# joshua16266261/self-play-ai

Hardware: AMD Instinct MI355X
Metric: MCTS sims/sec + self-play games/sec, Connect4 800 sims/move, 1/2/4/8 GPU (higher is better)
Workload: dtype bf16

## Files before the change

### self-play-ai_amd/csrc/net_c4.hip

```cpp
#include <algorithm>
#include <cmath>
#include <cstdlib>
#include <cstring>

#include "spai_internal.h"

namespace spai {
namespace {

typedef __bf16 bf16x8 __attribute__((ext_vector_type(8)));
typedef float f32x4 __attribute__((ext_vector_type(4)));
typedef float f32x2 __attribute__((ext_vector_type(2)));
typedef __bf16 bf16x2 __attribute__((ext_vector_type(2)));
typedef short i16x2 __attribute__((ext_vector_type(2)));

constexpr int kHid = 64;
constexpr int kS = 8;
constexpr int kP = kS * c4::kCells;
__host__ __device__ constexpr int npt_of(int S) { return (S * c4::kCells + 15) / 16; }
constexpr int kWaves = 4;
#ifdef SPAI_W8
constexpr int kPhysWaves = 8;
#else
constexpr int kPhysWaves = 4;
#endif
constexpr int kThreads = kPhysWaves * 64;
constexpr int kStemThreads = kWaves * 64;
constexpr int kKStepsRes = 18;
constexpr int kHeadC = 35;
constexpr int kPolIn = 32 * c4::kCells;
constexpr int kValIn = 3 * c4::kCells;

constexpr int kZ = 0;
constexpr int kX = 256;
constexpr int kZ1 = kX + kP * 128;
constexpr int kY = kZ1 + 256;
constexpr int kHC = 36;
constexpr int kLinFeat = kHC * 42;
constexpr int kLinK = 1536;
constexpr int kLinKSteps = kLinK / 32;
constexpr int kLinPitch = kLinK + 16;
constexpr int kLinHalves = 2;
constexpr int kLinBSteps = kLinKSteps / kLinHalves;
constexpr int kH = kY;
constexpr int kHBytes = kP * 128;
constexpr int kB = kH + kHBytes;
constexpr int kL = kB + kS * 16;
constexpr int kMaxBlocks = 20;
constexpr int kBiasFloats = kHid + 2 * kMaxBlocks * kHid + kHid;
constexpr int kBias = kL + kWaves * kLinHalves * 64 * 4;
constexpr int kBiasPer = (kBiasFloats + kStemThreads - 1) / kStemThreads;
constexpr int kPlanes = kBias + kBiasFloats * 4;
constexpr int kPlaneRow = 34;
constexpr int kWStem = kPlanes + kS * kPlaneRow * 8;
constexpr int kTab = kWStem + 4 * 64 * 16;
constexpr int kLinWPer = kLinBSteps / kWaves;
#ifdef SPAI_W8
constexpr int kSRun = 5;
constexpr int kSplitMaxN = 14;
constexpr int kPart = kTab + 42 * 16;
constexpr int kLdsBytes = kPart + kWaves * kSplitMaxN * 1024;
#else
constexpr int kSRun = kS;
constexpr int kLdsBytes = kTab + 42 * 16;
#endif
#ifdef SPAI_DIAG_KSTEP
constexpr int kStamps = 48;
#else
constexpr int kStamps = 24;
#endif
static_assert(kS * kLinPitch * 2 <= kHBytes, "head features fit in Y");
static_assert(kLdsBytes <= 160 * 1024, "LDS budget");

struct NetParams {
    const uint4 *w_stem;
    const uint4 *w_res;
    const uint4 *w_head;
    const float *b_conv;
    const uint4 *w_lin;
    const float *b_pol;
    const float *b_val;
    const uint4 *geo;
    const uint4 *lane_geo;
    unsigned long long *stamps;
    int blocks;
};

#ifdef SPAI_DIAG_HEAD
constexpr bool kDiagHead = true;
#else
constexpr bool kDiagHead = false;
#endif
#ifdef SPAI_DIAG_ENTRY
constexpr bool kDiagEntry = true;
#else
[[maybe_unused]] constexpr bool kDiagEntry = false;
#endif
__device__ __forceinline__ void stamp(const NetParams &P, int wave, int lane, int k) {
#ifdef SPAI_DIAG
    if (P.stamps && lane == 0 && wave >= 0) P.stamps[((size_t)blockIdx.x * kWaves + wave) * kStamps + k] = __builtin_amdgcn_s_memtime();
#endif
}
__device__ __forceinline__ void stamp_real(const NetParams &P, int wave, int lane, int k) {
#ifdef SPAI_DIAG
    if (P.stamps && lane == 0 && wave >= 0)
        P.stamps[((size_t)blockIdx.x * kWaves + wave) * kStamps + k] = __builtin_amdgcn_s_memrealtime();
#endif
}

__device__ __forceinline__ bf16x8 as_bf16x8(uint4 v) { return __builtin_bit_cast(bf16x8, v); }

__device__ __forceinline__ uint32_t pack_bf16x2(float a, float b) {
    return __builtin_bit_cast(uint32_t, __builtin_convertvector((f32x2){a, b}, bf16x2));
}

__device__ __forceinline__ uint32_t pack_relu_bf16x2(float a, float b) {
    const i16x2 h = __builtin_bit_cast(i16x2, __builtin_convertvector((f32x2){a, b}, bf16x2));
    return __builtin_bit_cast(uint32_t, __builtin_elementwise_max(h, (i16x2){0, 0}));
}

constexpr uint8_t kCellOrder[9][42] = {
    {0, 0, 0, 0, 0, 0, 0, 0, 0, 0, 0, 0, 0, 0, 0, 0, 0, 0, 0, 0, 0, 0, 0, 0, 0, 0, 0, 0, 0, 0, 0, 0, 0, 0, 0, 0, 0, 0, 0, 0, 0, 0},
    {0, 1, 2, 3, 4, 5, 6, 7, 8, 9, 10, 11, 12, 13, 14, 15, 16, 17, 18, 19, 20, 21, 22, 23, 24, 25, 26, 27, 28, 29, 30, 31, 32, 33, 34, 35, 36, 37, 38, 39, 40, 41},
    {0, 1, 2, 3, 4, 5, 6, 7, 8, 9, 10, 11, 12, 13, 14, 15, 16, 17, 18, 19, 20, 21, 22, 23, 24, 25, 26, 27, 28, 29, 30, 31, 32, 33, 34, 35, 36, 37, 38, 39, 40, 41},
    {0, 1, 2, 3, 4, 5, 6, 7, 8, 9, 10, 11, 12, 13, 14, 15, 16, 17, 18, 19, 20, 21, 22, 23, 24, 25, 26, 27, 28, 29, 30, 31, 32, 33, 34, 35, 36, 37, 38, 39, 40, 41},
    {22, 33, 10, 23, 24, 11, 26, 17, 8, 25, 18, 5, 6, 3, 4, 1, 34, 13, 20, 27, 30, 9, 16, 7, 38, 37, 40, 41, 0, 21, 14, 35, 32, 31, 12, 29, 28, 19, 2, 15, 36, 39},
    {13, 5, 30, 10, 23, 12, 38, 40, 37, 36, 0, 32, 27, 41, 20, 34, 2, 4, 3, 1, 16, 18, 26, 33, 39, 31, 22, 11, 28, 21, 14, 7, 8, 9, 15, 19, 24, 17, 35, 25, 29, 6},
    {37, 20, 40, 33, 22, 13, 25, 24, 35, 39, 38, 7, 10, 32, 19, 17, 27, 34, 41, 8, 16, 11, 36, 12, 2, 0, 4, 6, 26, 28, 1, 29, 30, 3, 15, 9, 31, 5, 23, 18, 21, 14},
    {8, 22, 4, 3, 1, 13, 20, 9, 33, 7, 21, 14, 25, 18, 19, 24, 35, 28, 0, 2, 5, 31, 32, 12, 16, 38, 36, 40, 39, 37, 26, 17, 27, 6, 34, 11, 30, 15, 23, 29, 10, 41},
    {28, 21, 41, 37, 18, 26, 1, 2, 16, 29, 22, 31, 15, 17, 5, 6, 24, 8, 13, 20, 4, 3, 33, 30, 27, 34, 0, 35, 12, 25, 23, 10, 36, 39, 19, 11, 32, 9, 38, 40, 7, 14},
};
__host__ __device__ constexpr uint16_t tap_skip(int S, int t) {
    constexpr uint16_t m1[21] = {0, 0, 0, 0, 0, 0, 0, 0, 0, 0, 0, 0, 0, 0, 0, 0, 0, 0, 0, 0, 0};
    constexpr uint16_t m2[21] = {0, 0, 0, 0, 0, 0, 0, 0, 0, 0, 0, 0, 0, 0, 0, 0, 0, 0, 0, 0, 0};
    constexpr uint16_t m3[21] = {0, 0, 0, 0, 0, 0, 0, 0, 0, 0, 0, 0, 0, 0, 0, 0, 0, 0, 0, 0, 0};
    constexpr uint16_t m4[21] = {0, 0, 0, 7, 292, 0, 448, 73, 0, 0, 448, 0, 0, 0, 0, 0, 0, 0, 0, 0, 0};
    constexpr uint16_t m5[21] = {0, 0, 448, 0, 292, 7, 0, 0, 0, 73, 0, 0, 0, 295, 0, 0, 0, 0, 0, 0, 0};
    constexpr uint16_t m6[21] = {256, 0, 0, 448, 0, 0, 292, 0, 0, 7, 0, 0, 0, 0, 0, 73, 0, 0, 0, 0, 0};
    constexpr uint16_t m7[21] = {0, 7, 4, 0, 73, 0, 0, 73, 7, 0, 0, 448, 448, 0, 292, 0, 0, 0, 484, 0, 0};
    constexpr uint16_t m8[21] = {73, 448, 0, 7, 0, 0, 0, 7, 0, 292, 7, 0, 292, 73, 0, 0, 448, 0, 0, 448, 73};
    return S == 1 ? m1[t] : S == 2 ? m2[t] : S == 3 ? m3[t] : S == 4 ? m4[t] : S == 5 ? m5[t] : S == 6 ? m6[t] : S == 7 ? m7[t] : m8[t];
}
__host__ __device__ constexpr bool cell_major(int S) { return S >= 4; }
__host__ __device__ constexpr int lin_pitch(int S) { return S == 4 ? 1552 : 1544; }
__host__ __device__ constexpr int first_kstep(int S, int t) {
    int tap = 0;
    while ((tap_skip(S, t) >> tap) & 1) ++tap;
    return 2 * tap;
}

#ifndef SPAI_CO_MAJOR_MAX_NPT
#define SPAI_CO_MAJOR_MAX_NPT 8
#endif
#ifndef SPAI_PAIR_MAX_NPT
#define SPAI_PAIR_MAX_NPT 11
#endif
#ifndef SPAI_HEAD_CO_MAJOR_MAX_NPT
#define SPAI_HEAD_CO_MAJOR_MAX_NPT 8
#endif
#ifdef SPAI_DEFER_EPI
constexpr bool kDefer = true;
#else
constexpr bool kDefer = false;
#endif
__host__ __device__ constexpr int kstep_of(int j) { return kDefer ? (j < 9 ? 2 * j : 2 * (j - 9) + 1) : j; }

template <int W, int CT, int NPT>
struct Plan {
    static constexpr int MODE = NPT <= (CT == 3 ? SPAI_HEAD_CO_MAJOR_MAX_NPT : SPAI_CO_MAJOR_MAX_NPT) ? 1
                                : CT == 4 && NPT <= SPAI_PAIR_MAX_NPT                              ? 2
                                                                                                    : 0;
    static constexpr int TT = NPT * CT;
    static constexpr int first = TT * W / 4;
    static constexpr int nr = TT * (W + 1) / 4 - first;
    static constexpr int last = first + nr - 1;
    static constexpr int m = NPT / 2, r = NPT % 2, pj = W >> 1, ph = W & 1;

    static constexpr int n = MODE == 2 ? 2 * m + r : nr;
    static constexpr int C0 = MODE == 2 ? 2 * pj : MODE == 1 ? first / NPT : 0;
    static constexpr int CTL = MODE == 2 ? 2 : MODE == 1 ? last / NPT - C0 + 1 : CT;
    static constexpr int T0 = MODE == 2 ? ph * m
                              : MODE == 1 ? (CTL == 1 ? first % NPT : 0)
                                          : first / CT;
    static constexpr int NT = MODE == 2 ? m + r : MODE == 1 ? (CTL == 1 ? nr : NPT) : last / CT - T0 + 1;
    static constexpr int gpt(int t) { return MODE == 2 && t == m ? NPT - 1 : T0 + t; }
    static constexpr int pt(int i) {
        return MODE == 2 ? (i < 2 * m ? i / 2 : m) : (MODE == 1 ? (first + i) % NPT : (first + i) / CT) - T0;
    }
    static constexpr int co(int i) {
        return MODE == 2 ? (i < 2 * m ? 2 * pj + (i & 1) : 2 * pj + ph)
                         : MODE == 1 ? (first + i) / NPT : (first + i) % CT;
    }
    static constexpr bool DEFER = kDefer && CT == 4 && MODE == 0;
    static constexpr int count_deferred() {
        int c = 0;
        for (int i = 0; i < n; ++i) c += co(i) >= 2;
        return c;
    }
    static constexpr int ND = DEFER ? count_deferred() : 0;
    static constexpr int NDA = ND > 0 ? n : 1;
    static constexpr bool deferred(int i) { return DEFER && co(i) >= 2; }
};

template <int NT>
struct Geo {
    uint32_t rel2[NT][5];
    int epi[NT];
    __device__ __forceinline__ uint32_t b(int t, int tap) const {
        return (tap & 1) ? rel2[t][tap >> 1] >> 16 : rel2[t][tap >> 1] & 0xFFFFu;
    }
};

struct RowCell {
    int s, cell, idx;
};
template <int S>
__device__ __forceinline__ RowCell row_cell(const uint8_t *smem, int p) {
    if (p >= S * c4::kCells) return RowCell{0, -1, 0};
    if constexpr (!cell_major(S)) {
        const int s = p / c4::kCells, cell = p - s * c4::kCells;
        return RowCell{s, cell, cell};
    } else {
        const int idx = p / S;
        return RowCell{p - idx * S, (int)((const uint32_t *)(smem + kTab))[idx * 4], idx};
    }
}

template <int W, int CT, int NPT, int S>
__device__ __forceinline__ void make_geo(const uint8_t *smem, int lane, Geo<Plan<W, CT, NPT>::NT> &g) {
    using PL = Plan<W, CT, NPT>;
    const int col = lane & 15, q = lane >> 4;
#pragma unroll
    for (int t = 0; t < PL::NT; ++t) {
        const int p = PL::gpt(t) * 16 + col;
        if constexpr (!cell_major(S)) {
            const int cell = p % c4::kCells;
            const int h = cell / c4::kCols, w = cell - h * c4::kCols;
#pragma unroll
            for (int tap = 0; tap < 9; ++tap) {
                const int dh = tap / 3 - 1, dw = tap % 3 - 1;
                const int r = p + dh * c4::kCols + dw;
                const bool ok = (unsigned)(h + dh) < (unsigned)c4::kRows && (unsigned)(w + dw) < (unsigned)c4::kCols;
                const int full = r * 128 + ((q ^ (r & 7)) << 4);
                const uint32_t v = (uint32_t)((ok ? full : (full & 255) - 256) + 256);
                if (tap & 1) g.rel2[t][tap >> 1] |= v << 16;
                else g.rel2[t][tap >> 1] = v;
            }
        } else {
            const bool real = p < S * c4::kCells;
            const int idx = real ? p / S : 0, s = p - idx * S;
            const uint4 e = *(const uint4 *)(smem + kTab + idx * 16);
            const int own = p * 128 + ((q ^ (p & 7)) << 4);
#pragma unroll
            for (int tap = 0; tap < 9; ++tap) {
                const uint32_t word = tap < 4 ? e.y : tap < 8 ? e.z : e.w;
                const int nb = (int)((word >> (8 * (tap & 3))) & 255u);
                int v;
                if (real && nb != 255) {
                    const int r = nb * S + s;
                    v = r * 128 + ((q ^ (r & 7)) << 4) + 256;
                } else if (S == 4) {
                    const int r = (((idx ^ (tap / 3 + tap % 3)) & 1) << 2) + s;
                    v = (r * 128 + ((q ^ (r & 7)) << 4)) & 255;
                } else {
                    v = own & 255;
                }
                if (tap & 1) g.rel2[t][tap >> 1] |= (uint32_t)v << 16;
                else g.rel2[t][tap >> 1] = (uint32_t)v;
            }
        }
        g.epi[t] = p * 128 + ((((q >> 1)) ^ (p & 7)) << 4) + ((q & 1) << 3);
    }
}

#ifndef SPAI_GEO_NT
#define SPAI_GEO_NT 8
#endif
constexpr int kGeoNT = SPAI_GEO_NT;
__host__ __device__ constexpr size_t lane_geo_at(int S, int W, int t) {
    return (((size_t)(S - 1) * kWaves + W) * kGeoNT + t) * 64 * 2;
}
constexpr size_t kLaneGeoU4 = lane_geo_at(kS + 1, 0, 0);

template <int W, int NPT, int S>
__device__ __forceinline__ void load_geo(const NetParams &P, int lane, Geo<Plan<W, 4, NPT>::NT> &g,
                                         int (&aux)[Plan<W, 4, NPT>::NT]) {
    constexpr int NT = Plan<W, 4, NPT>::NT;
    static_assert(NT <= kGeoNT, "lane geometry table depth");
    const uint4 *src = P.lane_geo + lane_geo_at(S, W, 0) + 2 * lane;
#pragma unroll
    for (int t = 0; t < NT; ++t) {
        const uint4 a = src[t * 128], b = src[t * 128 + 1];
        g.rel2[t][0] = a.x;
        g.rel2[t][1] = a.y;
        g.rel2[t][2] = a.z;
        g.rel2[t][3] = a.w;
        g.rel2[t][4] = b.x;
        g.epi[t] = (int)b.y;
        aux[t] = (int)b.z;
    }
}

template <int S, int W>
__device__ void geo_init_one(const uint8_t *smem, uint4 *out, int lane) {
    constexpr int NPT = npt_of(S);
    using PL = Plan<W, 4, NPT>;
    Geo<PL::NT> g;
    make_geo<W, 4, NPT, S>(smem, lane, g);
    uint4 *dst = out + lane_geo_at(S, W, 0) + 2 * lane;
    for (int t = 0; t < PL::NT; ++t) {
        const RowCell rc = row_cell<S>(smem, PL::gpt(t) * 16 + (lane & 15));
        const int h = rc.cell / c4::kCols, w = rc.cell - h * c4::kCols;
        const int aux = rc.cell < 0 ? S : rc.s | (w * 7 + h) << 8;
        dst[t * 128] = make_uint4(g.rel2[t][0], g.rel2[t][1], g.rel2[t][2], g.rel2[t][3]);
        dst[t * 128 + 1] = make_uint4(g.rel2[t][4], (uint32_t)g.epi[t], (uint32_t)aux, 0u);
    }
}

template <int S>
__device__ void geo_init_s(const uint8_t *smem, uint4 *out, int W, int lane) {
    if (W == 0) geo_init_one<S, 0>(smem, out, lane);
    else if (W == 1) geo_init_one<S, 1>(smem, out, lane);
    else if (W == 2) geo_init_one<S, 2>(smem, out, lane);
    else geo_init_one<S, 3>(smem, out, lane);
}

__global__ __launch_bounds__(64) void k_geo_init(const uint4 *__restrict__ geo, uint4 *__restrict__ out) {
    __shared__ __attribute__((aligned(16))) uint8_t smem[kLdsBytes];
    const int S = blockIdx.x / kWaves + 1, W = blockIdx.x % kWaves, lane = threadIdx.x;
    if (lane < c4::kCells) ((uint4 *)(smem + kTab))[lane] = geo[S * c4::kCells + lane];
    __syncthreads();
    switch (S) {
    case 1: geo_init_s<1>(smem, out, W, lane); break;
    case 2: geo_init_s<2>(smem, out, W, lane); break;
    case 3: geo_init_s<3>(smem, out, W, lane); break;
    case 4: geo_init_s<4>(smem, out, W, lane); break;
    case 5: geo_init_s<5>(smem, out, W, lane); break;
    case 6: geo_init_s<6>(smem, out, W, lane); break;
    case 7: geo_init_s<7>(smem, out, W, lane); break;
    default: geo_init_s<8>(smem, out, W, lane); break;
    }
}

#ifndef SPAI_FINAL_HINTS
#define SPAI_FINAL_HINTS 1
#endif
#ifndef SPAI_FINAL_FENCE
#define SPAI_FINAL_FENCE 1
#endif
#ifndef SPAI_ISSUE_HINTS
#define SPAI_ISSUE_HINTS 0
#endif
#ifndef SPAI_KSTEP_FENCE
#define SPAI_KSTEP_FENCE 1
#endif
#ifndef SPAI_DA4
#define SPAI_DA4 6
#endif
#ifndef SPAI_DB4
#define SPAI_DB4 2
#endif
#ifndef SPAI_DA8
#ifdef SPAI_FINAL2
#define SPAI_DA8 6
#else
#define SPAI_DA8 3
#endif
#endif
#ifndef SPAI_DB8
#define SPAI_DB8 3
#endif
__host__ __device__ constexpr int a_depth(int S) { return S <= 2 ? 9 : S <= 3 ? 6 : S <= 4 ? SPAI_DA4 : SPAI_DA8; }
__host__ __device__ constexpr int b_depth(int S) { return S <= 2 ? 4 : S <= 3 ? 3 : S <= 4 ? SPAI_DB4 : SPAI_DB8; }

__device__ __forceinline__ uint4 exp_a(const uint4 &src, int lane, int k) {
#ifdef SPAI_EXP_NOA
    (void)src;
    return make_uint4(0x3F803F80u ^ (uint32_t)(lane + k), 0x3F803F80u, 0x3F803F80u, (uint32_t)k);
#else
    (void)lane, (void)k;
    return src;
#endif
}
__device__ __forceinline__ uint4 exp_b(const uint8_t *p, int lane, int k) {
#ifdef SPAI_EXP_NOB
    (void)p;
    return make_uint4(0x3F803F80u ^ (uint32_t)(lane * 3 + k), 0x3F803F80u, 0x3F803F80u, (uint32_t)k);
#else
    (void)lane, (void)k;
    return *(const uint4 *)p;
#endif
}
__device__ __forceinline__ void layer_barrier() {
#ifndef SPAI_EXP_NOBAR
    __syncthreads();
#endif
}

template <int W, int CT, int NPT, int S, int DA, int DB, int EPI, int OUT>
__device__ __forceinline__ void final_tap_epilogue(uint8_t *smem, const Geo<Plan<W, CT, NPT>::NT> &g, int lane,
                                                   const uint4 (&A)[DA][Plan<W, CT, NPT>::CTL],
                                                   const uint4 (&B)[DB][Plan<W, CT, NPT>::NT],
                                                   const f32x4 (&bv)[Plan<W, CT, NPT>::CTL],
                                                   f32x4 (&acc)[Plan<W, CT, NPT>::n],
                                                   const int (&hoff)[Plan<W, CT, NPT>::NT],
                                                   f32x4 (&dacc)[Plan<W, CT, NPT>::NDA]) {
    using PL = Plan<W, CT, NPT>;
    auto defer = [](int i) { return EPI < 3 && PL::deferred(i); };
#ifdef SPAI_EXP_EPI_LAG
    constexpr int n = PL::n, k0 = kKStepsRes - 2, D = SPAI_EXP_EPI_LAG;
#else
    constexpr int n = PL::n, k0 = kKStepsRes - 2, D = 2;
#endif
    static_assert(CT == 4, "fused epilogue: 64-channel layers");
    auto live = [](int t, int ks) { return !((tap_skip(S, PL::gpt(t)) >> (ks >> 1)) & 1); };
    auto task_on = [](int i) { return !(EPI == 3 && PL::co(i) == 3); };
    uint4 id[2];
    uint4 rb[3];
    if (EPI == 2) {
        const int m = lane & 15, q = lane >> 4;
#pragma unroll
        for (int h = 0; h < 2; ++h) {
            const int j = 16 * h + m - 8 * q;
            uint32_t w[4];
#pragma unroll
            for (int e = 0; e < 4; ++e) w[e] = j == 2 * e ? 0x3F80u : j == 2 * e + 1 ? 0x3F800000u : 0u;
            id[h] = make_uint4(w[0], w[1], w[2], w[3]);
        }
#pragma unroll
        for (int i = 0; i < 2 && i < n; ++i)
            rb[i] = *(const uint4 *)(smem + (OUT - 256) + (g.b(PL::pt(i), 4) ^ ((PL::co(i) >> 1) << 6)));
    }
#pragma unroll
    for (int i = 0; i < n + D; ++i) {
        int nm = 0, nv = 0, nw = 0, nrd = 0;
        if (i < n) {
            if (EPI == 2 && i + 2 < n) {
                rb[(i + 2) % 3] = *(const uint4 *)(smem + (OUT - 256) + (g.b(PL::pt(i + 2), 4) ^ ((PL::co(i + 2) >> 1) << 6)));
                ++nrd;
            }
            const int t = PL::gpt(PL::pt(i)), c = PL::co(i) - PL::C0;
#pragma unroll
            for (int j = k0; j < kKStepsRes; ++j) {
                const int ks = kstep_of(j);
                if (task_on(i) && live(PL::pt(i), ks)) {
                    acc[i] = __builtin_amdgcn_mfma_f32_16x16x32_bf16(as_bf16x8(A[j % DA][c]), as_bf16x8(B[j % DB][PL::pt(i)]),
                                                                    ks == first_kstep(S, t) ? bv[c] : acc[i], 0, 0, 0);
                    ++nm;
                }
            }
            if (EPI == 2) {
                acc[i] = __builtin_amdgcn_mfma_f32_16x16x32_bf16(as_bf16x8(id[PL::co(i) & 1]), as_bf16x8(rb[i % 3]), acc[i],
                                                                0, 0, 0);
                ++nm;
            }
        }
        if (i >= D && EPI < 3 && !defer(i - D)) {
            const int j = i - D;
            const int off = OUT + (g.epi[PL::pt(j)] ^ (PL::co(j) << 5));
#if defined(SPAI_EXP_NOEPI) || defined(SPAI_EXP_NOEPI_ALL)
            asm volatile("" ::"a"(acc[j]));
#ifdef SPAI_EXP_NOEPI
            *(uint2 *)(smem + off) = make_uint2(0u, (uint32_t)off);
            nw = 1;
#endif
            nv = 0;
#elif defined(SPAI_EXP_STORE_B128)
            if ((j & 1) == 0) {
                const uint32_t a0 = pack_relu_bf16x2(acc[j][0], acc[j][1]), a1 = pack_relu_bf16x2(acc[j][2], acc[j][3]);
                const int j2 = j + 1 < PL::n ? j + 1 : j;
                const uint32_t b0 = pack_relu_bf16x2(acc[j2][0], acc[j2][1]), b1 = pack_relu_bf16x2(acc[j2][2], acc[j2][3]);
                *(uint4 *)(smem + (off & ~15)) = make_uint4(a0, a1, b0, b1);
                nw = 1;
            }
            nv = 5;
#elif defined(SPAI_EXP_STORE_LIN)
            (void)off;
            *(uint2 *)(smem + OUT + j * 512 + lane * 8) = make_uint2(pack_relu_bf16x2(acc[j][0], acc[j][1]),
                                                                     pack_relu_bf16x2(acc[j][2], acc[j][3]));
            nv = 5;
            nw = 1;
#else
            *(uint2 *)(smem + off) = make_uint2(pack_relu_bf16x2(acc[j][0], acc[j][1]), pack_relu_bf16x2(acc[j][2], acc[j][3]));
// ... 561 lines not shown
                if (i < CTL) __builtin_amdgcn_sched_group_barrier(0x020, 1, 0);
            }
        }
        __builtin_amdgcn_sched_barrier(0);
    }
    constexpr int h = (n + 1) / 2;
    constexpr int g0 = KH == 1 ? h : 0, g1 = KH == 1 ? n : h;
    constexpr int k0 = KH == 1 ? 0 : h, k1 = KH == 1 ? h : n;
    f32x4 *part = (f32x4 *)(smem + kPart) + (size_t)W * kSplitMaxN * 64 + lane;
#pragma unroll
    for (int i = g0; i < g1; ++i) part[i * 64] = acc[i];
    __syncthreads();
    uint4 id[2];
    if (EPI == 2) {
        const int m = lane & 15;
#pragma unroll
        for (int hh = 0; hh < 2; ++hh) {
            const int jj = 16 * hh + m - 8 * q;
            uint32_t wv[4];
#pragma unroll
            for (int e = 0; e < 4; ++e) wv[e] = jj == 2 * e ? 0x3F80u : jj == 2 * e + 1 ? 0x3F800000u : 0u;
            id[hh] = make_uint4(wv[0], wv[1], wv[2], wv[3]);
        }
    }
#pragma unroll
    for (int i = k0; i < k1; ++i) {
        const f32x4 p = part[i * 64];
        f32x4 a = KH == 1 ? acc[i] + p : p + acc[i];
        if (EPI == 2) {
            const uint4 rb = *(const uint4 *)(smem + (OUT - 256) + (g.b(PL::pt(i), 4) ^ ((PL::co(i) >> 1) << 6)));
            a = __builtin_amdgcn_mfma_f32_16x16x32_bf16(as_bf16x8(id[PL::co(i) & 1]), as_bf16x8(rb), a, 0, 0, 0);
        }
        const int off = OUT + (g.epi[PL::pt(i)] ^ (PL::co(i) << 5));
        *(uint2 *)(smem + off) = make_uint2(pack_relu_bf16x2(a[0], a[1]), pack_relu_bf16x2(a[2], a[3]));
    }
#else
    (void)smem, (void)g, (void)bias, (void)w, (void)wn, (void)lane, (void)A, (void)acc;
#endif
}

template <int KH, int CTL, int C0, int DA>
__device__ __forceinline__ void load_a_first_split(const uint4 *__restrict__ w, int lane, uint4 (&A)[DA][CTL]) {
#pragma unroll
    for (int j = 0; j < DA - 1; ++j)
#pragma unroll
        for (int c = 0; c < CTL; ++c) A[j][c] = w[((2 * j + KH - 1) * 4 + C0 + c) * 64 + lane];
}

template <int W, int S, bool FROM_X, int KH>
__device__ __forceinline__ void torso_and_heads(uint8_t *smem, const NetParams &P, const float *__restrict__ x,
                                                int base, int valid, int lane, const Geo<Plan<W, 4, npt_of(S)>::NT> &g,
                                                const int (&aux)[Plan<W, 4, npt_of(S)>::NT]) {
    constexpr int NPT = npt_of(S);
    using PL4 = Plan<W, 4, NPT>;
    constexpr size_t kLayer = (size_t)kKStepsRes * 4 * 64;
    const float *bias = (const float *)(smem + kBias);
    if constexpr (KH > 0) {
        constexpr int DA = 3, DB = b_depth(S), SW = KH == 2 ? -1 : W;
        uint4 A[DA][PL4::CTL];
        if (P.blocks > 0) load_a_first_split<KH, PL4::CTL, PL4::C0, DA>(P.w_res, lane, A);
        static_assert(!kDefer, "SPAI_W8 has no deferred epilogue");
        f32x4 dacc[PL4::NDA];
        if (KH == 1) stem<W, S, FROM_X>(smem, P, x, base, valid, lane, g, aux, dacc);
        __syncthreads();
        stamp(P, SW, lane, 1);
        for (int b = 0; b < P.blocks; ++b) {
            f32x4 acc[PL4::n];
            const int l1 = 2 * b, l2 = 2 * b + 1;
            conv_split<W, NPT, S, kX, DA, DB, 1, kY, KH>(smem, g, bias + kHid * (1 + l1), P.w_res + l1 * kLayer,
                                                        P.w_res + l2 * kLayer, lane, A, acc);
            layer_barrier();
            if (l1 < 12) stamp(P, SW, lane, 2 + l1);
            conv_split<W, NPT, S, kY, DA, DB, 2, kX, KH>(smem, g, bias + kHid * (1 + l2), P.w_res + l2 * kLayer,
                                                        b + 1 < P.blocks ? P.w_res + (l2 + 1) * kLayer : P.w_res + l2 * kLayer,
                                                        lane, A, acc);
            layer_barrier();
            if (l2 < 12) stamp(P, SW, lane, 2 + l2);
        }
        uint4 wlin[kLinWPer];
        if (KH == 1) {
            constexpr int DH = a_depth(S);
            uint4 Ah[DH][PL4::CTL];
            load_a_first<4, PL4::C0, PL4::CTL, DH>(P.w_head, lane, Ah);
            head_layer<W, S, DH>(smem, P, lane, g, aux, Ah, wlin, dacc);
        }
        __syncthreads();
        stamp(P, SW, lane, 14);
        if (KH == 1) linear_mfma<W, S>(smem, lane, wlin);
        return;
    }
    constexpr int DA = a_depth(S), DB = b_depth(S);
    uint4 A[DA][PL4::CTL];
    load_a_first<4, PL4::C0, PL4::CTL, DA>(P.blocks > 0 ? P.w_res : P.w_head, lane, A);
    f32x4 dacc[PL4::NDA];
    stem<W, S, FROM_X>(smem, P, x, base, valid, lane, g, aux, dacc);
    __syncthreads();
    stamp(P, W, lane, 1);
#ifdef SPAI_C4_BLOCK_UNROLL
#pragma unroll SPAI_C4_BLOCK_UNROLL
#endif
    for (int b = 0; b < P.blocks; ++b) {
        f32x4 acc[Plan<W, 4, NPT>::n];
        const int l1 = 2 * b, l2 = 2 * b + 1;
        unsigned long long *kst = nullptr;
#ifdef SPAI_DIAG_KSTEP
        if (b == 1 && P.stamps && lane == 0) kst = P.stamps + ((size_t)blockIdx.x * kWaves + W) * kStamps + 24;
#endif
        conv_mfma<W, 4, NPT, S, kX, DA, DB, 1, kY>(smem, g, bias + kHid * (1 + l1), P.w_res + l1 * kLayer,
                                                                    P.w_res + l2 * kLayer, lane, A, acc, aux, dacc, kst);
#ifdef SPAI_DIAG_KSTEP
        if (kst) kst[18] = __builtin_amdgcn_s_memtime();
#endif
#ifdef SPAI_DIAG
        if (b == 0 && !kDiagHead && !kDiagEntry) {
            asm volatile("" ::"v"(acc[0][0]), "v"(acc[PL4::n - 1][3]));
            stamp(P, W, lane, 17);
        }
#endif
#ifdef SPAI_DIAG
        if (b == 0 && !kDiagHead && !kDiagEntry) {
            asm volatile("s_waitcnt lgkmcnt(0)" ::: "memory");
            stamp(P, W, lane, 18);
        }
#endif
        layer_barrier();
#ifdef SPAI_DIAG_KSTEP
        if (kst) kst[19] = __builtin_amdgcn_s_memtime();
#endif
#ifdef SPAI_DIAG
        if (b == 0 && !kDiagHead && !kDiagEntry) stamp(P, W, lane, 19);
#endif
        if (l1 < 12) stamp(P, W, lane, 2 + l1);
        conv_mfma<W, 4, NPT, S, kY, DA, DB, 2, kX>(smem, g, bias + kHid * (1 + l2), P.w_res + l2 * kLayer,
                            b + 1 < P.blocks ? P.w_res + (l2 + 1) * kLayer : P.w_head, lane, A, acc, aux, dacc);
        layer_barrier();
        if (l2 < 12) stamp(P, W, lane, 2 + l2);
    }
    if (kDiagHead) stamp(P, W, lane, 19);
    uint4 wlin[kLinWPer];
    head_layer<W, S, DA>(smem, P, lane, g, aux, A, wlin, dacc);
    __syncthreads();
    stamp(P, W, lane, 14);
    linear_mfma<W, S>(smem, lane, wlin);
}

__host__ __device__ inline int group_size(uint32_t count, uint32_t grid) {
    const uint32_t cap = grid * (uint32_t)kSRun;
    const uint32_t rounds = count ? (count + cap - 1) / cap : 1u;
    const uint32_t per = grid * rounds;
    const int g = (int)((count + per - 1) / per);
    return g < 1 ? 1 : g > kSRun ? kSRun : g;
}

constexpr float kGroupCycles[kS + 1] = {0.f, 29200.f, 45500.f, 58600.f, 62900.f, 81200.f, 86200.f, 94700.f, 100500.f};
constexpr float kLaunchCycles = 4200.f;
#ifndef SPAI_CONC_CHAIN_CYCLES
#define SPAI_CONC_CHAIN_CYCLES 31000.f
#endif
#ifndef SPAI_CONC_MIN_COUNT
#define SPAI_CONC_MIN_COUNT 600
#endif
constexpr float kChainCycles = SPAI_CONC_CHAIN_CYCLES;
constexpr uint32_t kConcMinCount = SPAI_CONC_MIN_COUNT;
__host__ __device__ inline int group_size_conc(uint32_t count, uint32_t grid, int conc) {
    const int s0 = group_size(count, grid);
    if (conc <= 1 || count < kConcMinCount) return s0;
    float best = 3.0e38f;
    int bs = s0;
    for (int S = s0; S <= kSRun; ++S) {
        const uint32_t wgs = (count + S - 1) / S, rounds = (wgs + grid - 1) / grid;
        const float cu = (float)wgs * kGroupCycles[S] + (float)(wgs < grid ? wgs : grid) * kLaunchCycles;
        const float lat = (float)rounds * kGroupCycles[S] + kLaunchCycles;
        const float t = fmaxf((float)conc * cu / (float)grid, lat + kChainCycles);
        if (t < best) {
            best = t;
            bs = S;
        }
    }
    return bs;
}

template <int W, int S, bool FROM_X, int KH>
__device__ __forceinline__ void run_groups(uint8_t *smem, const NetParams &P, uint32_t count, int ngroups,
                                           const uint64_t *__restrict__ mine, const uint64_t *__restrict__ theirs,
                                           const float *__restrict__ x, float *__restrict__ priors,
                                           float *__restrict__ value, float *__restrict__ logits, int tid) {
    constexpr int wave = KH == 2 ? -1 : W;
    const int lane = tid & 63;
    for (int grp = blockIdx.x; grp < ngroups; grp += gridDim.x) {
        int ln = lane;
        asm volatile("" : "+v"(ln));
        ln &= 63;
        Geo<Plan<W, 4, npt_of(S)>::NT> g;
        int aux[Plan<W, 4, npt_of(S)>::NT];
        load_geo<W, npt_of(S), S>(P, ln, g, aux);
        const int base = grp * S;
        const int valid = min(S, (int)count - base);
        if (tid < kS) {
            uint64_t m = 0, t = 0;
            if (!FROM_X && tid < valid) {
                m = mine[base + tid];
                t = theirs[base + tid];
            }
            ((uint64_t *)(smem + kB))[2 * tid] = m;
            ((uint64_t *)(smem + kB))[2 * tid + 1] = t;
        }
#ifdef SPAI_DIAG_ENTRY
        if (grp == (int)blockIdx.x) {
            asm volatile("s_waitcnt vmcnt(0)" ::: "memory");
            stamp(P, wave, lane, 18);
        }
#endif
        if (!FROM_X && tid < kStemThreads) {
            const int s = tid >> 5, k = tid & 31;
            uint64_t v = 0;
            if (k < 27 && s < valid) {
                const uint64_t m = mine[base + s], t = theirs[base + s];
                const int tap = k / 3, ch = k - tap * 3;
                const uint64_t plane = ch == 0 ? m : ch == 1 ? t : (~(m | t) & c4::kBoard);
                const int off = (tap % 3 - 1) * 7 + (tap / 3 - 1);
                v = off >= 0 ? plane >> off : plane << -off;
            }
            ((uint64_t *)(smem + kPlanes))[s * kPlaneRow + k] = v;
        }
#ifdef SPAI_DIAG_ENTRY
        if (grp == (int)blockIdx.x) {
            asm volatile("s_waitcnt vmcnt(0) lgkmcnt(0)" ::: "memory");
            stamp(P, wave, lane, 19);
        }
#endif
        __syncthreads();
        stamp(P, wave, lane, 0);
        if (grp == (int)blockIdx.x) stamp_real(P, wave, lane, 22);
        torso_and_heads<W, S, FROM_X, KH>(smem, P, x, base, valid, ln, g, aux);
        __syncthreads();
        stamp(P, wave, lane, 15);
        if (tid < valid) {
            const float *L = (const float *)(smem + kL);
            const int slot = base + tid;
            float sum8[8];
#pragma unroll
            for (int o = 0; o < 8; ++o)
                sum8[o] = 0.f;
#pragma unroll
            for (int pp = 0; pp < kWaves * kLinHalves; ++pp)
#pragma unroll
                for (int o = 0; o < 8; ++o) sum8[o] += L[pp * 64 + tid * 8 + o];
            float lg[c4::kActions];
            float mx = -INFINITY;
#pragma unroll
            for (int a = 0; a < c4::kActions; ++a) {
                lg[a] = sum8[a] + P.b_pol[a];
                mx = fmaxf(mx, lg[a]);
            }
            const float v = tanhf(sum8[7] + P.b_val[0]);
            value[slot] = v;
            if (logits) {
#pragma unroll
                for (int a = 0; a < c4::kActions; ++a) logits[(size_t)slot * c4::kActions + a] = lg[a];
            }
            if (priors) {
                float e[c4::kActions], sum = 0.f;
#pragma unroll
                for (int a = 0; a < c4::kActions; ++a) {
                    e[a] = __expf(lg[a] - mx);
                    sum += e[a];
                }
                const float inv = 1.0f / sum;
#pragma unroll
                for (int a = 0; a < c4::kActions; ++a) e[a] *= inv;
                const uint64_t *bb = (const uint64_t *)(smem + kB);
                float out[c4::kActions];
                c4::mask_renorm(e, c4::open_columns(bb[2 * tid] | bb[2 * tid + 1]), out);
                float4 *pr = (float4 *)(priors + (size_t)slot * kPriorStride);
                pr[0] = make_float4(out[0], out[1], out[2], out[3]);
                pr[1] = make_float4(out[4], out[5], out[6], 0.f);
            }
        }
        stamp(P, wave, lane, 16);
        __syncthreads();
    }
}

template <int S, bool FROM_X>
__device__ __forceinline__ void dispatch_wave(uint8_t *smem, const NetParams &P, uint32_t count, int ngroups,
                                              const uint64_t *__restrict__ mine, const uint64_t *__restrict__ theirs,
                                              const float *__restrict__ x, float *__restrict__ priors,
                                              float *__restrict__ value, float *__restrict__ logits, int wave, int tid) {
#ifdef SPAI_W8
    constexpr int K0 = 1, K1 = 2;
#else
    constexpr int K0 = 0;
#endif
    switch (wave) {
    case 0: run_groups<0, S, FROM_X, K0>(smem, P, count, ngroups, mine, theirs, x, priors, value, logits, tid); break;
    case 1: run_groups<1, S, FROM_X, K0>(smem, P, count, ngroups, mine, theirs, x, priors, value, logits, tid); break;
    case 2: run_groups<2, S, FROM_X, K0>(smem, P, count, ngroups, mine, theirs, x, priors, value, logits, tid); break;
    case 3: run_groups<3, S, FROM_X, K0>(smem, P, count, ngroups, mine, theirs, x, priors, value, logits, tid); break;
#ifdef SPAI_W8
    case 4: run_groups<0, S, FROM_X, K1>(smem, P, count, ngroups, mine, theirs, x, priors, value, logits, tid); break;
    case 5: run_groups<1, S, FROM_X, K1>(smem, P, count, ngroups, mine, theirs, x, priors, value, logits, tid); break;
    case 6: run_groups<2, S, FROM_X, K1>(smem, P, count, ngroups, mine, theirs, x, priors, value, logits, tid); break;
    default: run_groups<3, S, FROM_X, K1>(smem, P, count, ngroups, mine, theirs, x, priors, value, logits, tid); break;
#else
    default: break;
#endif
    }
// ... 68 lines not shown
}

struct ConvRef {
    const float *w, *b, *bn;
    int ci, co;
};

void fold(const ConvRef &c, std::vector<float> &w, std::vector<float> &b) {
    w.assign((size_t)c.co * c.ci * 9, 0.f);
    b.assign(c.co, 0.f);
    for (int o = 0; o < c.co; ++o) {
        const float g = c.bn[o], be = c.bn[c.co + o], mu = c.bn[2 * c.co + o], var = c.bn[3 * c.co + o];
        const float scale = g / std::sqrt(var + 1e-5f);
        for (int i = 0; i < c.ci * 9; ++i) w[(size_t)o * c.ci * 9 + i] = c.w[(size_t)o * c.ci * 9 + i] * scale;
        b[o] = (c.b[o] - mu) * scale + be;
    }
}

}

size_t net_num_params(int game, int blocks, int hidden) {
    if (game != SPAI_GAME_CONNECT4) return 0;
    auto conv = [](size_t ci, size_t co) { return co * ci * 9 + co + 4 * co; };
    size_t n = conv(3, hidden) + (size_t)blocks * 2 * conv(hidden, hidden);
    n += conv(hidden, 32) + 7 * kPolIn + 7;
    n += conv(hidden, 3) + kValIn + 1;
    return n;
}

int net_create(spai_engine *e, int blocks, int hidden, const float *params, size_t nparams, int dtype,
               spai_net **out) {
    SPAI_CHECK(e->game == SPAI_GAME_CONNECT4, SPAI_ERR_UNSUPPORTED, "device net: only Connect4 is built");
    SPAI_CHECK(dtype == SPAI_DTYPE_BF16 || dtype == SPAI_DTYPE_F32, SPAI_ERR_INVALID, "unknown dtype %d", dtype);
    SPAI_CHECK(hidden == kHid, SPAI_ERR_UNSUPPORTED, "device net: hidden must be 64 (got %d)", hidden);
    SPAI_CHECK(blocks >= 0 && blocks <= kMaxBlocks, SPAI_ERR_UNSUPPORTED, "device net: 0..%d blocks (got %d)",
               kMaxBlocks, blocks);
    SPAI_CHECK(params && nparams == net_num_params(e->game, blocks, hidden), SPAI_ERR_INVALID,
               "expected %zu params, got %zu", net_num_params(e->game, blocks, hidden), nparams);
    if (dtype == SPAI_DTYPE_F32) {
        spai_net *n = new spai_net();
        n->eng = e;
        n->blocks = blocks;
        n->hidden = hidden;
        n->dtype = SPAI_DTYPE_F32;
        const int rc = net_create_f32(n, params);
        if (rc != SPAI_OK) {
            net_destroy(n);
            return rc;
        }
        *out = n;
        return SPAI_OK;
    }
    const float *p = params;
    auto take_conv = [&](int ci, int co) {
        ConvRef c{p, p + (size_t)co * ci * 9, p + (size_t)co * ci * 9 + co, ci, co};
        p += (size_t)co * ci * 9 + co + 4 * co;
        return c;
    };
    ConvRef stem_c = take_conv(3, kHid);
    std::vector<ConvRef> res;
    for (int i = 0; i < 2 * blocks; ++i) res.push_back(take_conv(kHid, kHid));
    ConvRef pol_c = take_conv(kHid, 32);
    const float *pol_w = p, *pol_b = p + 7 * kPolIn;
    p += 7 * kPolIn + 7;
    ConvRef val_c = take_conv(kHid, 3);
    const float *val_w = p, *val_b = p + kValIn;
    p += kValIn + 1;

    std::vector<float> fw, fb;
    std::vector<uint16_t> ws(4 * 64 * 8, 0);
    std::vector<float> bs(kHid);
    fold(stem_c, fw, fb);
    for (int ct = 0; ct < 4; ++ct)
        for (int l = 0; l < 64; ++l)
            for (int j = 0; j < 8; ++j) {
                int co = ct * 16 + (l & 15), k = 8 * (l >> 4) + j;
                float v = 0.f;
                if (k < 27) v = fw[(size_t)co * 27 + (k % 3) * 9 + k / 3];
                ws[(ct * 64 + l) * 8 + j] = f2bf(v);
            }
    for (int o = 0; o < kHid; ++o) bs[o] = fb[o];
    std::vector<uint16_t> wr((size_t)2 * blocks * kKStepsRes * 4 * 64 * 8);
    std::vector<float> br((size_t)2 * blocks * kHid);
    for (int L = 0; L < 2 * blocks; ++L) {
        fold(res[L], fw, fb);
        for (int ks = 0; ks < kKStepsRes; ++ks)
            for (int ct = 0; ct < 4; ++ct)
                for (int l = 0; l < 64; ++l)
                    for (int j = 0; j < 8; ++j) {
                        int co = ct * 16 + (l & 15), k = ks * 32 + 8 * (l >> 4) + j;
                        int tap = k / kHid, ci = k % kHid;
                        wr[((((size_t)L * kKStepsRes + ks) * 4 + ct) * 64 + l) * 8 + j] =
                            f2bf(fw[((size_t)co * kHid + ci) * 9 + tap]);
                    }
        for (int o = 0; o < kHid; ++o) br[(size_t)L * kHid + o] = fb[o];
    }
    std::vector<float> pw, pb, vw, vb;
    fold(pol_c, pw, pb);
    fold(val_c, vw, vb);
    std::vector<uint16_t> wh((size_t)kKStepsRes * 4 * 64 * 8, 0);
    std::vector<float> bh(kHid, 0.f);
    for (int ks = 0; ks < kKStepsRes; ++ks)
        for (int ct = 0; ct < 4; ++ct)
            for (int l = 0; l < 64; ++l)
                for (int j = 0; j < 8; ++j) {
                    int co = ct * 16 + (l & 15), k = ks * 32 + 8 * (l >> 4) + j;
                    int tap = k / kHid, ci = k % kHid;
                    float v = 0.f;
                    if (co < 32) v = pw[((size_t)co * kHid + ci) * 9 + tap];
                    else if (co < kHeadC) v = vw[((size_t)(co - 32) * kHid + ci) * 9 + tap];
                    wh[(((size_t)ks * 4 + ct) * 64 + l) * 8 + j] = f2bf(v);
                }
    for (int o = 0; o < 32; ++o) bh[o] = pb[o];
    for (int o = 0; o < 3; ++o) bh[32 + o] = vb[o];

    spai_net *n = new spai_net();
    n->eng = e;
    if (hipDeviceGetAttribute(&n->n_cu, hipDeviceAttributeMultiprocessorCount, e->device) != hipSuccess || n->n_cu < 1)
        n->n_cu = 256;
    n->blocks = blocks;
    n->hidden = hidden;
    int rc = SPAI_OK;
    auto up = [&](auto &buf, const auto &vec) {
        if (rc != SPAI_OK) return;
        rc = buf.alloc(vec.size());
        if (rc == SPAI_OK && !vec.empty() &&
            hipMemcpy(buf.p, vec.data(), vec.size() * sizeof(vec[0]), hipMemcpyHostToDevice) != hipSuccess) {
            set_error("hipMemcpy of net weights failed");
            rc = SPAI_ERR_DEVICE;
        }
    };
    up(n->w_stem, ws);
    if (blocks > 0) up(n->w_res, wr);
    up(n->w_head, wh);
    {
        std::vector<float> bc(bs);
        bc.insert(bc.end(), br.begin(), br.end());
        bc.insert(bc.end(), bh.begin(), bh.end());
        up(n->b_conv, bc);
    }
    std::vector<uint16_t> wlin((size_t)kLinBSteps * 64 * 8, 0);
    for (int ks = 0; ks < kLinBSteps; ++ks)
        for (int l = 0; l < 64; ++l)
            for (int j = 0; j < 8; ++j) {
                const int o = l & 7;
                const int k = ((l >> 3) & 1) * (kLinK / 2) + ks * 32 + 8 * (l >> 4) + j;
                const int cell = k / kHC, c = k % kHC;
                float v = 0.f;
                if (k < kLinFeat && o < 7 && c < 32) v = pol_w[(size_t)o * kPolIn + c * c4::kCells + cell];
                else if (k < kLinFeat && o == 7 && c >= 32 && c < kHeadC) v = val_w[(c - 32) * c4::kCells + cell];
                wlin[((size_t)ks * 64 + l) * 8 + j] = f2bf(v);
            }
    up(n->w_lin, wlin);
    std::vector<uint32_t> geo((size_t)9 * c4::kCells * 4, 0);
    for (int S = 1; S <= kS; ++S) {
        int idx_of[c4::kCells];
        for (int i = 0; i < c4::kCells; ++i) idx_of[kCellOrder[S][i]] = i;
        for (int i = 0; i < c4::kCells; ++i) {
            const int cell = kCellOrder[S][i], h = cell / c4::kCols, w = cell % c4::kCols;
            uint32_t *e = &geo[((size_t)S * c4::kCells + i) * 4];
            e[0] = (uint32_t)cell;
            for (int tap = 0; tap < 9; ++tap) {
                const int hh = h + tap / 3 - 1, ww = w + tap % 3 - 1;
                const bool ok = hh >= 0 && hh < c4::kRows && ww >= 0 && ww < c4::kCols;
                const uint32_t nb = ok ? (uint32_t)idx_of[hh * c4::kCols + ww] : 255u;
                e[1 + tap / 4] |= nb << (8 * (tap % 4));
            }
        }
    }
    up(n->geo, geo);
    if (rc == SPAI_OK) rc = n->lane_geo.alloc(kLaneGeoU4 * 4);
    if (rc == SPAI_OK) {
        k_geo_init<<<kS * kWaves, 64, 0, e->stream>>>((const uint4 *)n->geo.p, (uint4 *)n->lane_geo.p);
        if (hipGetLastError() != hipSuccess || hipStreamSynchronize(e->stream) != hipSuccess) {
            set_error("lane geometry kernel failed");
            rc = SPAI_ERR_DEVICE;
        }
    }
    up(n->b_pol, std::vector<float>(pol_b, pol_b + 7));
    up(n->b_val, std::vector<float>(val_b, val_b + 1));
    if (rc != SPAI_OK) {
        net_destroy(n);
        return rc;
    }
    *out = n;
    return SPAI_OK;
}

void net_destroy(spai_net *n) {
    if (!n) return;
    for (auto *b : {&n->w_stem, &n->w_res, &n->w_head, &n->w_lin}) b->release();
    for (auto *b : {&n->b_conv, &n->b_pol, &n->b_val, &n->f32, &n->io_x,
                    &n->io_logits, &n->io_value, &n->io_priors})
        b->release();
    n->io_mine.release();
    n->io_theirs.release();
    n->io_count.release();
    n->geo.release();
    n->lane_geo.release();
    delete n;
}

static NetParams params_of(const spai_net *n) {
    NetParams P;
    P.w_stem = (const uint4 *)n->w_stem.p;
    P.w_res = (const uint4 *)n->w_res.p;
    P.w_head = (const uint4 *)n->w_head.p;
    P.b_conv = n->b_conv.p;
    P.w_lin = (const uint4 *)n->w_lin.p;
    P.b_pol = n->b_pol.p;
    P.b_val = n->b_val.p;
    P.geo = (const uint4 *)n->geo.p;
    P.lane_geo = (const uint4 *)n->lane_geo.p;
    P.stamps = nullptr;
    P.blocks = n->blocks;
    return P;
}

int ensure_io(spai_net *n, uint32_t cnt) {
    if (n->io_value.n >= cnt) return SPAI_OK;
    SPAI_TRY(n->io_x.alloc((size_t)cnt * 126));
    SPAI_TRY(n->io_logits.alloc((size_t)cnt * 7));
    SPAI_TRY(n->io_value.alloc(cnt));
    SPAI_TRY(n->io_priors.alloc((size_t)cnt * kPriorStride));
    SPAI_TRY(n->io_mine.alloc(cnt));
    SPAI_TRY(n->io_theirs.alloc(cnt));
    return SPAI_OK;
}

static void random_positions(uint32_t cnt, std::vector<uint64_t> &m, std::vector<uint64_t> &t) {
    m.resize(cnt);
    t.resize(cnt);
    uint64_t h = 0x1234;
    for (uint32_t i = 0; i < cnt; ++i) {
        c4::State s{0, 0, 0, c4::kOngoing};
        h = c4::splitmix64(h);
        for (int k = 0, plies = (int)(h % 30); k < plies; ++k) {
            uint32_t lm = c4::legal_mask(s.x, s.o, s.status);
            h = c4::splitmix64(h);
            c4::State r;
            c4::next_state(s, c4::kth_bit(lm, (int)(h % c4::popc32(lm))), r);
            if (r.status != c4::kOngoing) break;
            s = r;
        }
        const bool xm = c4::x_to_move(s.n);
        m[i] = xm ? s.x : s.o;
        t[i] = xm ? s.o : s.x;
    }
}

int net_bench(spai_net *n, uint32_t cnt, uint32_t iters, double *ms, int conc) {
    SPAI_CHECK(cnt > 0 && iters > 0, SPAI_ERR_INVALID, "need cnt > 0 and iters > 0");
    SPAI_TRY(ensure_io(n, cnt));
    if (!n->io_count.p) SPAI_TRY(n->io_count.alloc(1));
    hipStream_t st = n->eng->stream;
    std::vector<uint64_t> m, t;
    random_positions(cnt, m, t);
    SPAI_HIP(hipMemcpyAsync(n->io_mine.p, m.data(), (size_t)cnt * 8, hipMemcpyHostToDevice, st));
    SPAI_HIP(hipMemcpyAsync(n->io_theirs.p, t.data(), (size_t)cnt * 8, hipMemcpyHostToDevice, st));
    SPAI_HIP(hipMemcpyAsync(n->io_count.p, &cnt, 4, hipMemcpyHostToDevice, st));
    for (int w = 0; w < 3; ++w)
        SPAI_TRY(net_eval_batch(n, st, n->io_count.p, cnt, n->io_mine.p, n->io_theirs.p, n->io_priors.p, n->io_value.p,
                                0, conc));
    hipEvent_t a, b;
    SPAI_HIP(hipEventCreate(&a));
    SPAI_HIP(hipEventCreate(&b));
    SPAI_HIP(hipEventRecord(a, st));
    for (uint32_t i = 0; i < iters; ++i)
        SPAI_TRY(net_eval_batch(n, st, n->io_count.p, cnt, n->io_mine.p, n->io_theirs.p, n->io_priors.p, n->io_value.p,
                                0, conc));
    SPAI_HIP(hipEventRecord(b, st));
    SPAI_HIP(hipEventSynchronize(b));
    float f = 0;
    SPAI_HIP(hipEventElapsedTime(&f, a, b));
    (void)hipEventDestroy(a);
    (void)hipEventDestroy(b);
    *ms = f / iters;
    return SPAI_OK;
}

int net_phase_stamps(spai_net *n, uint32_t cnt, double *cycles) {
#ifndef SPAI_DIAG
    (void)n;
    (void)cycles;
    SPAI_CHECK(false, SPAI_ERR_UNSUPPORTED, "phase stamps need the diagnostic build (make -C self-play-ai_amd diag)");
#endif
    SPAI_CHECK(cnt > 0, SPAI_ERR_INVALID, "need cnt > 0");
    SPAI_CHECK(n->dtype == SPAI_DTYPE_BF16, SPAI_ERR_UNSUPPORTED, "phase stamps time the bf16 kernel");
    SPAI_TRY(ensure_io(n, cnt));
    hipStream_t st = n->eng->stream;
    std::vector<uint64_t> m, t;
    random_positions(cnt, m, t);
    const char *es = std::getenv("SPAI_PHASE_S");
    const int S = es ? std::max(1, std::min(kSRun, std::atoi(es))) : kSRun;
    uint32_t grid = (cnt + S - 1) / S;
    if (const char *eg = std::getenv("SPAI_PHASE_GRID"))
        grid = std::min<uint32_t>(grid, (uint32_t)std::max(1, std::atoi(eg)));
    DevBuf<unsigned long long> d;
    SPAI_TRY(d.alloc((size_t)grid * kWaves * kStamps));
    SPAI_HIP(hipMemsetAsync(d.p, 0, d.n * 8, st));
    SPAI_HIP(hipMemcpyAsync(n->io_mine.p, m.data(), (size_t)cnt * 8, hipMemcpyHostToDevice, st));
    SPAI_HIP(hipMemcpyAsync(n->io_theirs.p, t.data(), (size_t)cnt * 8, hipMemcpyHostToDevice, st));
    NetParams P = params_of(n);
    P.stamps = d.p;
    for (int rep = 0; rep < 3; ++rep)
        k_forward<false><<<grid, kThreads, 0, st>>>(nullptr, cnt, S, 1, n->io_mine.p, n->io_theirs.p, nullptr, P,
                                                   n->io_priors.p, n->io_value.p, nullptr);
    SPAI_HIP(hipGetLastError());
    std::vector<unsigned long long> hs(d.n);
    SPAI_HIP(hipMemcpyAsync(hs.data(), d.p, d.n * 8, hipMemcpyDeviceToHost, st));
    SPAI_HIP(hipStreamSynchronize(st));
    for (int k = 0; k < kStamps; ++k) cycles[k] = 0;
    double cntw = 0;
    unsigned long long first_in = ~0ull, last_out = 0;
    for (uint32_t g = 0; g < grid; ++g)
        for (int w = 0; w < kWaves; ++w) {
            const unsigned long long *sp = hs.data() + ((size_t)g * kWaves + w) * kStamps;
            if (!sp[0] || !sp[16]) continue;
            for (int k = 0; k < 20; ++k) cycles[k] += sp[k] ? (double)(long long)(sp[k] - sp[0]) : 0.0;
// ... 92 lines not shown
```

Measured before the change: 69.96 million.

## Use searched row permutation tables for S=2,3 to skip zero conv taps

For group sizes 2 and 3, rows are placed by a precomputed permutation table (kRowTab) instead of the linear sample-major layout. This lets whole 16-row tiles share out-of-board neighbours, so tap_skip masks can drop those conv k-steps. The geometry init builds per-row neighbour tables for these sizes, and padding rows map to a safe zero-ish offset. The cost model cycles for S=2,3 are lowered to match, which may shift group-size choices.

```diff
diff --git a/self-play-ai_amd/csrc/net_c4.hip b/self-play-ai_amd/csrc/net_c4.hip
--- a/self-play-ai_amd/csrc/net_c4.hip
+++ b/self-play-ai_amd/csrc/net_c4.hip
@@ -54,6 +54,7 @@
 constexpr int kPlaneRow = 34;
 constexpr int kWStem = kPlanes + kS * kPlaneRow * 8;
 constexpr int kTab = kWStem + 4 * 64 * 16;
+constexpr int kTabRows = 128;
 constexpr int kLinWPer = kLinBSteps / kWaves;
 #ifdef SPAI_W8
 constexpr int kSRun = 5;
@@ -130,10 +131,15 @@
     {8, 22, 4, 3, 1, 13, 20, 9, 33, 7, 21, 14, 25, 18, 19, 24, 35, 28, 0, 2, 5, 31, 32, 12, 16, 38, 36, 40, 39, 37, 26, 17, 27, 6, 34, 11, 30, 15, 23, 29, 10, 41},
     {28, 21, 41, 37, 18, 26, 1, 2, 16, 29, 22, 31, 15, 17, 5, 6, 24, 8, 13, 20, 4, 3, 33, 30, 27, 34, 0, 35, 12, 25, 23, 10, 36, 39, 19, 11, 32, 9, 38, 40, 7, 14},
 };
+constexpr uint8_t kRowTab[2][128] = {
+    {13, 54, 12, 58, 11, 52, 10, 51, 9, 50, 8, 53, 16, 57, 15, 55, 0, 255, 255, 44, 6, 47, 5, 46, 4, 45, 3, 48, 2, 43, 1, 42, 37, 78, 36, 77, 39, 80, 38, 83, 41, 82, 40, 81, 35, 255, 255, 79, 23, 64, 22, 67, 20, 61, 19, 60, 18, 59, 17, 62, 25, 66, 24, 65, 14, 255, 255, 49, 21, 255, 255, 70, 28, 255, 255, 63, 7, 255, 255, 56, 32, 73, 31, 76, 30, 71, 29, 69, 27, 68, 26, 72, 34, 75, 33, 74, 255, 255, 255, 255, 255, 255, 255, 255, 255, 255, 255, 255, 255, 255, 255, 255, 255, 255, 255, 255, 255, 255, 255, 255, 255, 255, 255, 255, 255, 255, 255, 255},
+    {45, 5, 2, 44, 86, 46, 88, 85, 0, 87, 47, 89, 4, 1, 43, 3, 16, 50, 18, 23, 12, 9, 22, 11, 8, 29, 10, 15, 57, 17, 30, 19, 40, 37, 79, 39, 81, 123, 83, 125, 122, 82, 124, 121, 36, 78, 38, 80, 32, 66, 71, 52, 65, 25, 51, 64, 24, 58, 26, 31, 73, 33, 59, 72, 98, 21, 63, 7, 49, 91, 112, 35, 77, 42, 84, 105, 28, 70, 14, 56, 61, 95, 100, 68, 94, 54, 67, 93, 53, 74, 92, 60, 102, 99, 75, 101, 69, 13, 34, 76, 118, 41, 104, 48, 90, 111, 55, 97, 20, 62, 6, 27, 114, 119, 116, 255, 110, 107, 96, 109, 106, 103, 108, 113, 255, 115, 120, 117},
+};
+constexpr int8_t kRowLin[2][2] = {{4, 6}, {3, 5}};
 __host__ __device__ constexpr uint16_t tap_skip(int S, int t) {
     constexpr uint16_t m1[21] = {0, 0, 0, 0, 0, 0, 0, 0, 0, 0, 0, 0, 0, 0, 0, 0, 0, 0, 0, 0, 0};
-    constexpr uint16_t m2[21] = {0, 0, 0, 0, 0, 0, 0, 0, 0, 0, 0, 0, 0, 0, 0, 0, 0, 0, 0, 0, 0};
-    constexpr uint16_t m3[21] = {0, 0, 0, 0, 0, 0, 0, 0, 0, 0, 0, 0, 0, 0, 0, 0, 0, 0, 0, 0, 0};
+    constexpr uint16_t m2[21] = {0, 7, 448, 0, 73, 0, 0, 0, 0, 0, 0, 0, 0, 0, 0, 0, 0, 0, 0, 0, 0};
+    constexpr uint16_t m3[21] = {7, 0, 448, 0, 73, 0, 292, 0, 0, 0, 0, 0, 0, 0, 0, 0, 0, 0, 0, 0, 0};
     constexpr uint16_t m4[21] = {0, 0, 0, 7, 292, 0, 448, 73, 0, 0, 448, 0, 0, 0, 0, 0, 0, 0, 0, 0, 0};
     constexpr uint16_t m5[21] = {0, 0, 448, 0, 292, 7, 0, 0, 0, 73, 0, 0, 0, 295, 0, 0, 0, 0, 0, 0, 0};
     constexpr uint16_t m6[21] = {256, 0, 0, 448, 0, 0, 292, 0, 0, 7, 0, 0, 0, 0, 0, 73, 0, 0, 0, 0, 0};
@@ -142,6 +148,8 @@
     return S == 1 ? m1[t] : S == 2 ? m2[t] : S == 3 ? m3[t] : S == 4 ? m4[t] : S == 5 ? m5[t] : S == 6 ? m6[t] : S == 7 ? m7[t] : m8[t];
 }
 __host__ __device__ constexpr bool cell_major(int S) { return S >= 4; }
+__host__ __device__ constexpr bool row_table(int S) { return S == 2 || S == 3; }
+__host__ __device__ constexpr int geo_rows_at(int S) { return 9 * c4::kCells + (S - 2) * kTabRows; }
 __host__ __device__ constexpr int lin_pitch(int S) { return S == 4 ? 1552 : 1544; }
 __host__ __device__ constexpr int first_kstep(int S, int t) {
     int tap = 0;
@@ -216,6 +224,10 @@
 };
 template <int S>
 __device__ __forceinline__ RowCell row_cell(const uint8_t *smem, int p) {
+    if constexpr (row_table(S)) {
+        const uint32_t e = ((const uint32_t *)(smem + kTab))[p * 4];
+        return e == ~0u ? RowCell{0, -1, 0} : RowCell{(int)(e & 255u), (int)(e >> 8), 0};
+    }
     if (p >= S * c4::kCells) return RowCell{0, -1, 0};
     if constexpr (!cell_major(S)) {
         const int s = p / c4::kCells, cell = p - s * c4::kCells;
@@ -233,7 +245,24 @@
 #pragma unroll
     for (int t = 0; t < PL::NT; ++t) {
         const int p = PL::gpt(t) * 16 + col;
-        if constexpr (!cell_major(S)) {
+        if constexpr (row_table(S)) {
+            const uint4 e = *(const uint4 *)(smem + kTab + p * 16);
+            const bool real = e.x != ~0u;
+#pragma unroll
+            for (int tap = 0; tap < 9; ++tap) {
+                const uint32_t word = tap < 4 ? e.y : tap < 8 ? e.z : e.w;
+                const int nb = (int)((word >> (8 * (tap & 3))) & 255u);
+                int v;
+                if (real && nb != 255) {
+                    v = nb * 128 + ((q ^ (nb & 7)) << 4) + 256;
+                } else {
+                    const int r = (p + kRowLin[S - 2][0] * (tap / 3 - 1) + kRowLin[S - 2][1] * (tap % 3 - 1)) & 7;
+                    v = (r * 128 + ((q ^ r) << 4)) & 255;
+                }
+                if (tap & 1) g.rel2[t][tap >> 1] |= (uint32_t)v << 16;
+                else g.rel2[t][tap >> 1] = (uint32_t)v;
+            }
+        } else if constexpr (!cell_major(S)) {
             const int cell = p % c4::kCells;
             const int h = cell / c4::kCols, w = cell - h * c4::kCols;
 #pragma unroll
@@ -326,9 +355,13 @@
 }
 
 __global__ __launch_bounds__(64) void k_geo_init(const uint4 *__restrict__ geo, uint4 *__restrict__ out) {
-    __shared__ __attribute__((aligned(16))) uint8_t smem[kLdsBytes];
+    __shared__ __attribute__((aligned(16))) uint8_t smem[kTab + kTabRows * 16];
     const int S = blockIdx.x / kWaves + 1, W = blockIdx.x % kWaves, lane = threadIdx.x;
-    if (lane < c4::kCells) ((uint4 *)(smem + kTab))[lane] = geo[S * c4::kCells + lane];
+    if (row_table(S)) {
+        for (int r = lane; r < kTabRows; r += 64) ((uint4 *)(smem + kTab))[r] = geo[geo_rows_at(S) + r];
+    } else if (lane < c4::kCells) {
+        ((uint4 *)(smem + kTab))[lane] = geo[S * c4::kCells + lane];
+    }
     __syncthreads();
     switch (S) {
     case 1: geo_init_s<1>(smem, out, W, lane); break;
@@ -1196,7 +1229,7 @@
     return g < 1 ? 1 : g > kSRun ? kSRun : g;
 }
 
-constexpr float kGroupCycles[kS + 1] = {0.f, 29200.f, 45500.f, 58600.f, 62900.f, 81200.f, 86200.f, 94700.f, 100500.f};
+constexpr float kGroupCycles[kS + 1] = {0.f, 29000.f, 43500.f, 52000.f, 62900.f, 81200.f, 86200.f, 94700.f, 100500.f};
 constexpr float kLaunchCycles = 4200.f;
 #ifndef SPAI_CONC_CHAIN_CYCLES
 #define SPAI_CONC_CHAIN_CYCLES 31000.f
@@ -1571,7 +1604,7 @@
                 wlin[((size_t)ks * 64 + l) * 8 + j] = f2bf(v);
             }
     up(n->w_lin, wlin);
-    std::vector<uint32_t> geo((size_t)9 * c4::kCells * 4, 0);
+    std::vector<uint32_t> geo((size_t)geo_rows_at(4) * 4, 0);
     for (int S = 1; S <= kS; ++S) {
         int idx_of[c4::kCells];
         for (int i = 0; i < c4::kCells; ++i) idx_of[kCellOrder[S][i]] = i;
@@ -1584,6 +1617,27 @@
                 const bool ok = hh >= 0 && hh < c4::kRows && ww >= 0 && ww < c4::kCols;
                 const uint32_t nb = ok ? (uint32_t)idx_of[hh * c4::kCols + ww] : 255u;
                 e[1 + tap / 4] |= nb << (8 * (tap % 4));
+            }
+        }
+    }
+    for (int S = 2; S <= 3; ++S) {
+        int row_of[3 * c4::kCells];
+        for (int r = 0; r < npt_of(S) * 16; ++r)
+            if (kRowTab[S - 2][r] != 255) row_of[kRowTab[S - 2][r]] = r;
+        for (int r = 0; r < kTabRows; ++r) {
+            uint32_t *e = &geo[((size_t)geo_rows_at(S) + r) * 4];
+            const int code = kRowTab[S - 2][r];
+            e[0] = ~0u;
+            e[1] = e[2] = e[3] = ~0u;
+            if (code == 255) continue;
+            const int s = code / c4::kCells, cell = code % c4::kCells, h = cell / c4::kCols, w = cell % c4::kCols;
+            e[0] = (uint32_t)s | (uint32_t)cell << 8;
+            for (int tap = 0; tap < 9; ++tap) {
+                const int hh = h + tap / 3 - 1, ww = w + tap % 3 - 1;
+                const bool ok = hh >= 0 && hh < c4::kRows && ww >= 0 && ww < c4::kCols;
+                if (!ok) continue;
+                const uint32_t nb = (uint32_t)row_of[s * c4::kCells + hh * c4::kCols + ww], sh = 8 * (tap % 4);
+                e[1 + tap / 4] = (e[1 + tap / 4] & ~(255u << sh)) | nb << sh;
             }
         }
     }
```

Measured after the change: 71.23 million, median of 6. 1.8% higher.
